# sharinka0715/semantic-gaussians

Measured on NVIDIA B200. Metric: Mviews/s + HBM GB/s, 1M Gaussians, 256-ch features, 1080p, fwd+bwd, higher is better.
Workload: dtype f32

## Files before the change

### semantic-gaussians_b200/csrc/blend_v3.cu

```cuda
#include <cstdlib>
#include <cstring>
#include <cuda.h>
#include "common.cuh"
#include "blend_pool.cuh"

namespace sgb {

namespace {

constexpr int kThreads = SGB_TILE_PIX;

__device__ __forceinline__ int lane_group8(int lane) { return (lane & 1) | (((lane >> 2) & 3) << 1); }
__device__ __forceinline__ int lane_group4(int lane) { return ((lane >> 1) & 1) | ((lane >> 4) << 1); }

template <int N>
__device__ __forceinline__ void xreduce_step(float (&v)[8], int lane, int step) {
    const bool upper = (lane & step) != 0;
#pragma unroll
    for (int i = 0; i < N / 2; i++) {
        const float send = upper ? v[i] : v[i + N / 2];
        const float keep = upper ? v[i + N / 2] : v[i];
        v[i] = keep + __shfl_xor_sync(0xffffffffu, send, step);
    }
}

constexpr int kAB = 32;

struct __align__(16) AlphaSmem {
    float4 recA[kAB];
    float4 recB[kAB];
    uint32_t ids[kAB];
    float wbuf[kAB][SGB_TILE_PIX];
    uint32_t wmask[8];
    uint32_t slot_chunk[kAB];
    uint32_t cur_chunk;
    uint32_t s_last;
};

template <bool DEPTH>
__global__ void __launch_bounds__(kThreads) alpha_pass_kernel(
    const uint2* __restrict__ ranges, const uint32_t* __restrict__ point_list, int W, int H,
    const SplatRec* __restrict__ rec, float* __restrict__ final_T, uint32_t* __restrict__ n_contrib,
    uint32_t* __restrict__ tile_last, float* __restrict__ out_depth, PoolView pool) {
    extern __shared__ __align__(128) unsigned char smem_raw[];
    AlphaSmem& sm = *reinterpret_cast<AlphaSmem*>(smem_raw);

    const int tiles_x = (W + SGB_TILE - 1) / SGB_TILE;
    const int tile = blockIdx.x;
    const int tid = threadIdx.x, lane = tid & 31, warp = tid >> 5;
    const uint32_t tx = tid & (SGB_TILE - 1), ty = tid >> 4;
    const uint2 pix = {(uint32_t)(tile % tiles_x) * SGB_TILE + tx, (uint32_t)(tile / tiles_x) * SGB_TILE + ty};
    const uint32_t pix_id = W * pix.y + pix.x;
    const float2 pixf = {(float)pix.x, (float)pix.y};
    const bool inside = pix.x < (uint32_t)W && pix.y < (uint32_t)H;
    bool done = !inside;

    const uint2 range = ranges[tile];
    const int total = (int)(range.y - range.x);
    const int nbatches = (total + kAB - 1) / kAB;
    const uint32_t dbase = range.x / kChunkEntries + (uint32_t)tile;
    if (tid == 0) { sm.cur_chunk = kNone; sm.s_last = 0; }

    float T = 1.0f;
    uint32_t last_contributor = 0;
    float D = 15.0f;
    uint32_t n_tile = 0;
    uint32_t n_blend = 0;

    auto load_id = [&](int bb) -> uint32_t {
        const int i = bb * kAB + tid;
        return (tid < kAB && bb < nbatches && i < total) ? __ldg(point_list + range.x + i) : 0u;
    };
    uint32_t id_cur = load_id(0), id_nxt = load_id(1);
    float4 rA = make_float4(0.f, 0.f, 0.f, 0.f), rB = rA;
    if (tid < kAB && tid < total) {
        const float4* rp = reinterpret_cast<const float4*>(rec + id_cur);
        rA = __ldg(rp);
        rB = __ldg(rp + 1);
    }
    for (int b = 0; b < nbatches; b++) {
        const int num_done = __syncthreads_count(done);
        if (num_done == kThreads) break;
        const int base = b * kAB;
        const int cnt = min(kAB, total - base);
        if (tid < cnt) {
            sm.ids[tid] = id_cur;
            sm.recA[tid] = rA;
            sm.recB[tid] = rB;
        }
        __syncthreads();
        if (tid < kAB) {
            id_cur = id_nxt;
            if (base + kAB + tid < total) {
                const float4* rp = reinterpret_cast<const float4*>(rec + id_cur);
                rA = __ldg(rp);
                rB = __ldg(rp + 1);
            }
            id_nxt = load_id(b + 2);
        }
        uint32_t my_mask = 0;
        for (int j = 0; j < cnt; j++) {
            float w = 0.f;
            if (!done) {
                const float4 a = sm.recA[j];
                const float2 xy = {a.x, a.y};
                const float2 d = {xy.x - pixf.x, xy.y - pixf.y};
                const float4 con_o = sm.recB[j];
                const float power = -0.5f * (con_o.x * d.x * d.x + con_o.z * d.y * d.y) - con_o.y * d.x * d.y;
                if (!(power > 0.0f)) {
                    const float alpha = min(0.99f, con_o.w * exp(power));
                    if (!(alpha < 1.0f / 255.0f)) {
                        const float test_T = T * (1 - alpha);
                        if (test_T < 0.0001f) {
                            done = true;
                        } else {
                            w = alpha * T;
                            if (DEPTH) {
                                if (T > 0.5f && test_T < 0.5) D = a.z;
                            }
                            T = test_T;
                            last_contributor = (uint32_t)(base + j + 1);
                        }
                    }
                }
            }
            sm.wbuf[j][tid] = w;
            n_blend += (w != 0.f);
            if (__ballot_sync(0xffffffffu, w != 0.f)) my_mask |= 1u << j;
        }
        if (lane == 0) sm.wmask[warp] = my_mask;
        __syncthreads();
        uint32_t tm = 0;
#pragma unroll
        for (int q = 0; q < 8; q++) tm |= sm.wmask[q];
        const int n_act = __popc(tm);
        if (n_act) {
            if (tid == 0) {
                uint32_t e = n_tile, cur = sm.cur_chunk;
                for (int k = 0; k < n_act; k++, e++) {
                    if ((e & (kChunkEntries - 1)) == 0) {
                        uint32_t nw = atomicAdd(&pool.hdr->counter, 1u);
                        if (nw >= pool.capacity) {
                            pool.hdr->overflow = 1;
                            nw = pool.capacity - 1;
                        }
                        pool.dir[dbase + e / kChunkEntries] = nw;
                        cur = nw;
                    }
                    sm.slot_chunk[k] = cur;
                }
                sm.cur_chunk = cur;
            }
            __syncthreads();
            int k = 0;
            for (uint32_t m = tm; m; m &= m - 1, k++) {
                const int j = __ffs(m) - 1;
                const uint32_t e = n_tile + k;
                WChunk& ck = pool.chunks[sm.slot_chunk[k]];
                const int s = e & (kChunkEntries - 1);
                ck.w[s][tid] = sm.wbuf[j][tid];
                if (tid == 0) {
                    uint32_t strips = 0;
#pragma unroll
                    for (int q = 0; q < 8; q++) strips |= ((sm.wmask[q] >> j) & 1u) << q;
                    ck.meta[s] = make_uint2(sm.ids[j], strips);
                }
// ... 199 lines not shown
    struct Stage {
        float w[ES][SGB_TILE_PIX];
        float f[ES][CH];
    };
    extern __shared__ __align__(128) unsigned char smem_raw[];
    Stage* stg = reinterpret_cast<Stage*>(smem_raw);
    __shared__ uint64_t full_bar[NS], empty_bar[NS];
    __shared__ uint32_t Cdir[kDirCap];
    __shared__ __align__(16) float Tsm[SGB_TILE_PIX];
    __shared__ float bgS[CH];

    const int tiles_x = (W + SGB_TILE - 1) / SGB_TILE;
    const int nchunksC = (C + CH - 1) / CH;
    const int tile = blockIdx.x / nchunksC;
    const int ch0 = (blockIdx.x % nchunksC) * CH;
    const int nch = min(CH, C - ch0);
    const int tid = threadIdx.x, lane = tid & 31, warp = tid >> 5;
    const int pg = lane_group4(lane), cg = lane_group8(lane);
    const uint2 pix_min = {(uint32_t)(tile % tiles_x) * SGB_TILE, (uint32_t)(tile / tiles_x) * SGB_TILE};

    const uint32_t n = pool.count[tile];
    const int nb = (int)((n + ES - 1) / ES);
    const uint32_t dbase = pool.dirbase[tile];
    if (tid == 0) {
        for (int i = 0; i < NS; i++) {
            mbar_init(&full_bar[i], 1);
            mbar_init(&empty_bar[i], kThreads / 32);
        }
        mbar_fence_init();
    }
    for (int k = tid; k < min(nb, kDirCap); k += kThreads) Cdir[k] = chunk_of(pool, dbase, k);
    {
        const uint32_t x = pix_min.x + (tid & (SGB_TILE - 1)), y = pix_min.y + (tid >> 4);
        Tsm[tid] = (x < (uint32_t)W && y < (uint32_t)H) ? final_T[(size_t)W * y + x] : 0.f;
        if (tid < nch) bgS[tid] = bg_color[ch0 + tid];
    }
    if (nch < CH)
        for (int e = tid; e < NS * ES * CH; e += kThreads) {
            const int k = e % CH;
            if (k >= nch) stg[e / (ES * CH)].f[(e / CH) % ES][k] = 0.f;
        }
    __syncthreads();

    auto chunk_ptr = [&](int bi) {
        return pool.chunks + (bi < kDirCap ? Cdir[bi] : chunk_of(pool, dbase, bi));
    };
    auto load_meta = [&](int bi) {
        uint2 m = make_uint2(0u, 0u);
        if (bi < nb && lane < min(ES, (int)n - bi * ES)) m = __ldg(&chunk_ptr(bi)->meta[lane]);
        return m;
    };
    auto issue = [&](int bi, uint2 meta) {
        const int st = bi % NS;
        const int cnt = min(ES, (int)n - bi * ES);
        if (bi >= NS) mbar_wait(&empty_bar[st], (uint32_t)(((bi / NS) - 1) & 1));
        if (lane < cnt) {
            const WChunk* ck = chunk_ptr(bi);
            bulk_g2s(&stg[st].w[lane][0], &ck->w[lane][0], SGB_TILE_PIX * 4u, &full_bar[st]);
            bulk_g2s(&stg[st].f[lane][0], features + (size_t)meta.x * C + ch0, (uint32_t)nch * 4u, &full_bar[st]);
        }
        __syncwarp();
        if (lane == 0) mbar_arrive_expect_tx(&full_bar[st], (uint32_t)cnt * (SGB_TILE_PIX * 4u + (uint32_t)nch * 4u));
    };
    uint2 meta_next = make_uint2(0u, 0u);
    int pb = 0;
    if (warp == 0) {
        uint2 m[LA];
#pragma unroll
        for (int i = 0; i < LA; i++) m[i] = load_meta(i);
#pragma unroll
        for (int i = 0; i < LA; i++)
            if (i < nb) issue(i, m[i]);
        pb = min(LA, nb);
        meta_next = load_meta(pb);
    }

    float2 acc[8][MCH / 2];
#pragma unroll
    for (int i = 0; i < 8; i++)
#pragma unroll
        for (int k = 0; k < MCH / 2; k++) acc[i][k] = make_float2(0.f, 0.f);

    const int woff = warp * 32 + pg * 8;
    auto entry = [&](const Stage& sg, int e) {
        const float4 w0 = *reinterpret_cast<const float4*>(&sg.w[e][woff]);
        const float4 w1 = *reinterpret_cast<const float4*>(&sg.w[e][woff + 4]);
        float2 f[MCH / 2];
#pragma unroll
        for (int q = 0; q < MCH / 4; q++) {
            const float4 t = *reinterpret_cast<const float4*>(&sg.f[e][q * 32 + cg * 4]);
            f[2 * q] = make_float2(t.x, t.y);
            f[2 * q + 1] = make_float2(t.z, t.w);
        }
        const float wv[8] = {w0.x, w0.y, w0.z, w0.w, w1.x, w1.y, w1.z, w1.w};
#pragma unroll
        for (int i = 0; i < 8; i++) {
            const float2 w2 = make_float2(wv[i], wv[i]);
#pragma unroll
            for (int k = 0; k < MCH / 2; k++) acc[i][k] = ffma2(f[k], w2, acc[i][k]);
        }
    };
    for (int b = 0; b < nb; b++) {
        const int st = b % NS;
        const int cnt = min(ES, (int)n - b * ES);
        if (warp == 0 && pb < nb) {
            issue(pb, meta_next);
            pb++;
            meta_next = load_meta(pb);
        }
        mbar_wait(&full_bar[st], (uint32_t)((b / NS) & 1));
        if (cnt == ES) {
#pragma unroll
            for (int e = 0; e < ES; e++) entry(stg[st], e);
        } else {
            for (int e = 0; e < cnt; e++) entry(stg[st], e);
        }
        __syncwarp();
        if (lane == 0) mbar_arrive(&empty_bar[st]);
    }
    const uint32_t row = pix_min.y + 2 * warp + (pg >> 1);
    const uint32_t col0 = pix_min.x + (pg & 1) * 8;
    if (acc_nonfinite<MCH>(acc)) {
        forward_redo_guarded<MCH, true>(pool, n, dbase, features, C, ch0, nch, warp, woff, cg, bg_color, final_T, W, H,
                                        row, col0, out_color);
        return;
    }
    if (row < (uint32_t)H) {
        const size_t plane = (size_t)H * W;
        const bool vec = ((W & 3) == 0) && (col0 + 8 <= (uint32_t)W);
        const float4 t0 = *reinterpret_cast<const float4*>(&Tsm[(2 * warp + (pg >> 1)) * SGB_TILE + (pg & 1) * 8]);
        const float4 t1 = *reinterpret_cast<const float4*>(&Tsm[(2 * warp + (pg >> 1)) * SGB_TILE + (pg & 1) * 8 + 4]);
        const float Tv[8] = {t0.x, t0.y, t0.z, t0.w, t1.x, t1.y, t1.z, t1.w};
#pragma unroll
        for (int k = 0; k < MCH; k++) {
            const int chl = (k >> 2) * 32 + cg * 4 + (k & 3);
            if (chl >= nch) continue;
            const float bgc = bgS[chl];
            float* dst = out_color + (size_t)(ch0 + chl) * plane + (size_t)W * row + col0;
            float o[8];
#pragma unroll
            for (int i = 0; i < 8; i++) o[i] = ((k & 1) ? acc[i][k / 2].y : acc[i][k / 2].x) + Tv[i] * bgc;
            if (vec) {
                reinterpret_cast<float4*>(dst)[0] = make_float4(o[0], o[1], o[2], o[3]);
                reinterpret_cast<float4*>(dst)[1] = make_float4(o[4], o[5], o[6], o[7]);
            } else {
#pragma unroll
                for (int i = 0; i < 8; i++)
                    if (col0 + i < (uint32_t)W) dst[i] = o[i];
            }
        }
    }
}

template <int CH>
__global__ void __launch_bounds__(kThreads, 2) dfeature_gemm_kernel(int W, int H, int C,
                                                                   const float* __restrict__ dL_dpixels,
                                                                   PoolView pool, float* __restrict__ dL_dcolors) {
    static_assert(CH == 64, "64-channel chunks");
    constexpr int DP = SGB_TILE_PIX;
    constexpr int WP = 36;
    extern __shared__ __align__(128) unsigned char smem_raw[];
    float(*dLs)[DP] = reinterpret_cast<float(*)[DP]>(smem_raw);
    float* wslab = reinterpret_cast<float*>(smem_raw + sizeof(float) * CH * DP);
    __shared__ const float* Wrow[128];
    __shared__ uint32_t Gid[128];

    const int tiles_x = (W + SGB_TILE - 1) / SGB_TILE;
    const int nchunksC = (C + CH - 1) / CH;
    const int tile = blockIdx.x / nchunksC;
    const int ch0 = (blockIdx.x % nchunksC) * CH;
    const int nch = min(CH, C - ch0);
    const int tid = threadIdx.x, lane = tid & 31, warp = tid >> 5;
    const uint32_t n = pool.count[tile];
    if (n == 0) return;
    const uint32_t dbase = __ldg(pool.dirbase + tile);
    const uint2 pix_min = {(uint32_t)(tile % tiles_x) * SGB_TILE, (uint32_t)(tile / tiles_x) * SGB_TILE};
    const size_t plane = (size_t)H * W;
    const bool rows16 = (W & 3) == 0 && (reinterpret_cast<uintptr_t>(dL_dpixels) & 15) == 0;
    for (int idx = tid; idx < CH * SGB_TILE * 4; idx += kThreads) {
        const int pc = idx & 3, r = (idx >> 2) & (SGB_TILE - 1), c = idx >> 6;
        const uint32_t y = pix_min.y + r, x = pix_min.x + pc * 4;
        float* dst = &dLs[c][((r * 4 + pc) ^ ((c >> 2) & 7)) * 4];
        const float* src = dL_dpixels + (size_t)(ch0 + c) * plane + (size_t)W * y + x;
        const bool rowok = c < nch && y < (uint32_t)H;
        if (rows16) {
            const bool ok = rowok && x + 4 <= (uint32_t)W;
            cp_async16(dst, ok ? src : dL_dpixels, ok ? 16 : 0);
        } else {
#pragma unroll
            for (int i = 0; i < 4; i++) dst[i] = (rowok && x + i < (uint32_t)W) ? __ldg(src + i) : 0.f;
        }
    }
    cp_async_commit();

    const int eg = lane_group4(lane), cg = lane_group8(lane);
    const bool red16 = ((C & 3) == 0) && ((reinterpret_cast<uintptr_t>(dL_dcolors) & 15) == 0);
    for (uint32_t base = 0; base < n; base += 128) {
        const int cnt = (int)min(128u, n - base);
        __syncthreads();
        if (tid < cnt) {
            const WChunk* ck = pool.chunks + chunk_of(pool, dbase, (int)((base + tid) / kChunkEntries));
            const int s = (base + tid) & (kChunkEntries - 1);
            Wrow[tid] = &ck->w[s][0];
            Gid[tid] = ck->meta[s].x;
        }
        cp_async_wait<0>();
        __syncthreads();
        if (warp * 16 < cnt) {
            float(*wsl)[16][WP] = reinterpret_cast<float(*)[16][WP]>(wslab + (size_t)warp * 2 * 16 * WP);
            const float* lrow[4];
#pragma unroll
            for (int i = 0; i < 4; i++) lrow[i] = Wrow[min(warp * 16 + (lane >> 3) + 4 * i, cnt - 1)] + (lane & 7) * 4;
            auto issue = [&](int sl, int buf) {
#pragma unroll
                for (int i = 0; i < 4; i++)
                    cp_async16(&wsl[buf][(lane >> 3) + 4 * i][(lane & 7) * 4], lrow[i] + sl * 32, 16);
                cp_async_commit();
            };
            float2 acc[4][8];
#pragma unroll
            for (int j = 0; j < 4; j++)
#pragma unroll
                for (int k = 0; k < 8; k++) acc[j][k] = make_float2(0.f, 0.f);
            issue(0, 0);
            for (int sl = 0; sl < SGB_TILE_PIX / 32; sl++) {
                const int buf = sl & 1;
                if (sl + 1 < SGB_TILE_PIX / 32) { issue(sl + 1, buf ^ 1); cp_async_wait<1>(); }
                else cp_async_wait<0>();
                __syncwarp();
                const float* drow = &dLs[4 * cg][0];
                const float* wbase = &wsl[buf][eg][0];
                auto ld_d = [&](int step) {
                    const int k = step & 7, p4 = step >> 3;
                    return *reinterpret_cast<const float4*>(drow + ((k >> 2) * 32 + (k & 3)) * DP +
                                                            (((sl * 8 + p4) ^ cg) << 2));
                };
                float4 wq[4], wn[4];
#pragma unroll
                for (int j = 0; j < 4; j++) wq[j] = *reinterpret_cast<const float4*>(wbase + 4 * j * WP);
                float4 d0 = ld_d(0), d1 = ld_d(1);
#pragma unroll
                for (int p4 = 0; p4 < 8; p4++) {
#pragma unroll
                    for (int k = 0; k < 8; k++) {
                        const int step = p4 * 8 + k;
                        float4 d2 = d1;
                        if (step + 2 < 64) d2 = ld_d(step + 2);
                        if (k == 2 && p4 + 1 < 8) {
#pragma unroll
                            for (int j = 0; j < 4; j++)
                                wn[j] = *reinterpret_cast<const float4*>(wbase + 4 * j * WP + (p4 + 1) * 4);
                        }
#pragma unroll
                        for (int j = 0; j < 4; j++) {
                            acc[j][k] = ffma2(make_float2(wq[j].x, wq[j].y), make_float2(d0.x, d0.y), acc[j][k]);
                            acc[j][k] = ffma2(make_float2(wq[j].z, wq[j].w), make_float2(d0.z, d0.w), acc[j][k]);
                        }
                        d0 = d1;
                        d1 = d2;
                    }
                    if (p4 + 1 < 8) {
#pragma unroll
                        for (int j = 0; j < 4; j++) wq[j] = wn[j];
                    }
                }
                __syncwarp();
            }
#pragma unroll
            for (int j = 0; j < 4; j++) {
                const int e = warp * 16 + eg + 4 * j;
                if (e < cnt) {
                    float* dst = dL_dcolors + (size_t)Gid[e] * C + ch0 + 4 * cg;
#pragma unroll
                    for (int h = 0; h < 2; h++) {
                        const int chl = h * 32 + 4 * cg;
                        const float4 v = make_float4(acc[j][4 * h + 0].x + acc[j][4 * h + 0].y, acc[j][4 * h + 1].x + acc[j][4 * h + 1].y,
                                                     acc[j][4 * h + 2].x + acc[j][4 * h + 2].y, acc[j][4 * h + 3].x + acc[j][4 * h + 3].y);
                        if (red16 && chl + 4 <= nch) {
                            red_add_v4_f32(dst + h * 32, v);
                        } else {
                            if (chl + 0 < nch) red_add_f32(dst + h * 32 + 0, v.x);
                            if (chl + 1 < nch) red_add_f32(dst + h * 32 + 1, v.y);
                            if (chl + 2 < nch) red_add_f32(dst + h * 32 + 2, v.z);
                            if (chl + 3 < nch) red_add_f32(dst + h * 32 + 3, v.w);
                        }
                    }
                }
            }
        }
    }
}

template <bool VEC>
__global__ void __launch_bounds__(kThreads, 2) chain_backward_gemm_kernel(
    int W, int H, int C, const float* __restrict__ bg_color, const SplatRec* __restrict__ rec,
    const float* __restrict__ features, const float* __restrict__ final_Ts, const float* __restrict__ dL_dpixels,
    PoolView pool, float* __restrict__ dL_dmean2D, float* __restrict__ dL_dconic2D, float* __restrict__ dL_dopacity) {
    constexpr int CK = 16;
    constexpr int FP = kSeg + 4;
    extern __shared__ __align__(128) unsigned char smem_raw[];
    float(*S)[kSeg][32] = reinterpret_cast<float(*)[kSeg][32]>(smem_raw);
    float(*FT)[CK][FP] = reinterpret_cast<float(*)[CK][FP]>(smem_raw + sizeof(float) * 8 * kSeg * 32);
    float(*DS)[2][CK][32] = reinterpret_cast<float(*)[2][CK][32]>(
        smem_raw + sizeof(float) * (8 * kSeg * 32 + 2 * CK * FP));
    __shared__ const float* Wrow[kSeg];
    __shared__ uint2 Meta[kSeg];
    __shared__ float4 RecA[kSeg], RecB[kSeg];

    const int tiles_x = (W + SGB_TILE - 1) / SGB_TILE;
    const int tile = blockIdx.x;
    const int tid = threadIdx.x, lane = tid & 31, warp = tid >> 5;
    const int pg = lane >> 3, eg = lane & 7;
    const uint2 pix_min = {(uint32_t)(tile % tiles_x) * SGB_TILE, (uint32_t)(tile / tiles_x) * SGB_TILE};
    const uint32_t tx = tid & (SGB_TILE - 1), ty = tid >> 4;
    const uint2 pix = {pix_min.x + tx, pix_min.y + ty};
    const uint32_t pix_id = W * pix.y + pix.x;
    const float2 pixf = {(float)pix.x, (float)pix.y};
    const bool inside = pix.x < (uint32_t)W && pix.y < (uint32_t)H;
    const uint32_t n = pool.count[tile];
    if (n == 0) return;
    const uint32_t dbase = pool.dirbase[tile];

    const size_t plane = (size_t)H * W;
    const bool rows16 = ((W & 3) == 0) && ((reinterpret_cast<uintptr_t>(dL_dpixels) & 15) == 0);
    const int woff = warp * 32 + lane;

    int bg_nonzero = 0;
    for (int ch = tid; ch < C; ch += kThreads) bg_nonzero |= (bg_color[ch] != 0.f);
    bg_nonzero = __syncthreads_or(bg_nonzero);
    float bgdot = 0.f;
    if (inside && bg_nonzero)
        for (int ch = 0; ch < C; ch++) bgdot += bg_color[ch] * __ldg(dL_dpixels + (size_t)ch * plane + pix_id);

    const float T_final = inside ? final_Ts[pix_id] : 0.f;
    float T = T_final;
    float last_alpha = 0.f, s_last = 0.f, A = 0.f;
    const float ddelx_dx = 0.5f * W, ddely_dy = 0.5f * H;

    const int nseg = (int)((n + kSeg - 1) / kSeg);
    for (int sg = nseg - 1; sg >= 0; sg--) {
        const int base = sg * kSeg;
        const int cnt = min(kSeg, (int)n - base);
        __syncthreads();
        if (tid < kSeg) {
            if (tid < cnt) {
                const WChunk* ck = pool.chunks + chunk_of(pool, dbase, (base + tid) / kChunkEntries);
                const int s = (base + tid) & (kChunkEntries - 1);
                Wrow[tid] = &ck->w[s][0];
                const uint2 mt = ck->meta[s];
                Meta[tid] = mt;
                const float4* rp = reinterpret_cast<const float4*>(rec + mt.x);
                RecA[tid] = __ldg(rp);
                RecB[tid] = __ldg(rp + 1);
            } else {
                Meta[tid] = make_uint2(0u, 0u);
            }
        }
        __syncthreads();

        float2 acc[8][4];
#pragma unroll
        for (int i = 0; i < 8; i++)
#pragma unroll
            for (int j = 0; j < 4; j++) acc[i][j] = make_float2(0.f, 0.f);

        const int nslab = (C + CK - 1) / CK;
        float4 fpre;
        auto fload = [&](int sl) {
            const int e = tid >> 2, q = tid & 3;
            const int chb = sl * CK + q * 4;
            fpre = make_float4(0.f, 0.f, 0.f, 0.f);
            if (e < cnt) {
                const float* src = features + (size_t)Meta[e].x * C + chb;
                if (VEC && chb + 4 <= C) fpre = __ldg(reinterpret_cast<const float4*>(src));
                else {
                    if (chb < C) fpre.x = __ldg(src);
                    if (chb + 1 < C) fpre.y = __ldg(src + 1);
                    if (chb + 2 < C) fpre.z = __ldg(src + 2);
                    if (chb + 3 < C) fpre.w = __ldg(src + 3);
                }
            }
        };
        auto fstore = [&](int buf) {
            const int e = tid >> 2, q = tid & 3;
            const int pos = ((e >> 3) << 2) | (e & 3) | (((e >> 2) & 1) << 5);
            FT[buf][q * 4 + 0][pos] = fpre.x;
            FT[buf][q * 4 + 1][pos] = fpre.y;
            FT[buf][q * 4 + 2][pos] = fpre.z;
            FT[buf][q * 4 + 3][pos] = fpre.w;
        };
        auto dissue = [&](int sl, int buf) {
#pragma unroll
            for (int i = 0; i < CK / 4; i++) {
                const int chl = (lane >> 3) + 4 * i;
                const int ch = sl * CK + chl;
                const int pc = lane & 7;
                const uint32_t y = pix_min.y + 2 * warp + (pc >> 2);
                const uint32_t x = pix_min.x + (pc & 3) * 4;
                const bool rowin = ch < C && y < (uint32_t)H;
                const float* src = dL_dpixels + (size_t)ch * plane + (size_t)W * y + x;
                if (rows16) {
                    const bool ok = rowin && x + 4 <= (uint32_t)W;
                    cp_async16(&DS[warp][buf][chl][pc * 4], ok ? src : dL_dpixels, ok ? 16 : 0);
                } else {
#pragma unroll
                    for (int u = 0; u < 4; u++)
                        DS[warp][buf][chl][pc * 4 + u] = (rowin && x + u < (uint32_t)W) ? __ldg(src + u) : 0.f;
                }
            }
            cp_async_commit();
        };
        fload(0);
        dissue(0, 0);
        fstore(0);
        if (nslab > 1) fload(1);
        for (int sl = 0; sl < nslab; sl++) {
            const int buf = sl & 1;
            if (sl + 1 < nslab) { dissue(sl + 1, buf ^ 1); cp_async_wait<1>(); }
            else cp_async_wait<0>();
            __syncthreads();
#pragma unroll 4
            for (int k = 0; k < CK; k++) {
                const float4 d0 = *reinterpret_cast<const float4*>(&DS[warp][buf][k][pg * 8]);
                const float4 d1 = *reinterpret_cast<const float4*>(&DS[warp][buf][k][pg * 8 + 4]);
                const float4 f0 = *reinterpret_cast<const float4*>(&FT[buf][k][eg * 4]);
                const float4 f1 = *reinterpret_cast<const float4*>(&FT[buf][k][32 + eg * 4]);
                const float2 ff[4] = {make_float2(f0.x, f0.y), make_float2(f0.z, f0.w), make_float2(f1.x, f1.y),
                                      make_float2(f1.z, f1.w)};
                const float d[8] = {d0.x, d0.y, d0.z, d0.w, d1.x, d1.y, d1.z, d1.w};
#pragma unroll
                for (int i = 0; i < 8; i++) {
                    const float2 d2 = make_float2(d[i], d[i]);
#pragma unroll
                    for (int j = 0; j < 4; j++) acc[i][j] = ffma2(ff[j], d2, acc[i][j]);
                }
            }
            if (sl + 1 < nslab) {
                fstore(buf ^ 1);
                if (sl + 2 < nslab) fload(sl + 2);
            }
            __syncwarp();
        }
#pragma unroll
// ... 635 lines not shown
    return guess;
}

static int launch_alpha_pass(sgb_ctx* ctx, const sgb_view_inputs& in, GeomView g, BinView b, ImgView im,
                             float* out_depth, const PoolView& pv, cudaStream_t s) {
    const int tiles = num_tiles(in);
    const size_t smem = sizeof(AlphaSmem);
    static DeviceOnce attr_set;
    if (attr_set.first_use_on_device()) {
        SGB_CUDA(cudaFuncSetAttribute(alpha_pass_kernel<false>, cudaFuncAttributeMaxDynamicSharedMemorySize, (int)smem));
        SGB_CUDA(cudaFuncSetAttribute(alpha_pass_kernel<true>, cudaFuncAttributeMaxDynamicSharedMemorySize, (int)smem));
    }
    SGB_CUDA(cudaMemsetAsync(pv.hdr, 0, sizeof(PoolHdr), s));
    StageTimer t(ctx, ST_ALPHA, s);
    if (out_depth)
        alpha_pass_kernel<true><<<tiles, kThreads, smem, s>>>(im.ranges, b.point_list, in.W, in.H, g.rec, im.final_T,
                                                            im.n_contrib, im.tile_last, out_depth, pv);
    else
        alpha_pass_kernel<false><<<tiles, kThreads, smem, s>>>(im.ranges, b.point_list, in.W, in.H, g.rec, im.final_T,
                                                             im.n_contrib, im.tile_last, nullptr, pv);
    SGB_LAUNCH_CHECK("alpha_pass_kernel", in.debug, s);
    ctx->launches += 1;
    return SGB_OK;
}

static int launch_forward_gemm(sgb_ctx* ctx, const sgb_view_inputs& in, ImgView im, const float* colors,
                               float* out_color, const PoolView& pv, cudaStream_t s) {
    const int tiles = num_tiles(in);
    const int chunks = (in.C + 63) / 64;
    const bool vec = (in.C % 4 == 0) && ((reinterpret_cast<uintptr_t>(colors) & 15) == 0);
    if (vec && blend_mma_enabled()) return launch_forward_mma(ctx, in, im, colors, out_color, pv, s);
    static const bool use_warp = [] { const char* e = getenv("SGB_FWD_WARP"); return e && e[0] == '1'; }();
    StageTimer t(ctx, ST_BLEND_FWD, s);
    ctx->launches += 1;
    if (use_warp) {
        const int nslices = (in.C + 31) / 32;
        const int SL = nslices >= 4 ? 4 : nslices;
        const int groups = (nslices + SL - 1) / SL;
        const size_t smem_w = sizeof(FwdWarpSmem) * (kThreads / 32);
        if (vec)
            blend_forward_warp_kernel<true><<<tiles * groups, kThreads, smem_w, s>>>(in.W, in.H, in.C, SL, colors, in.background,
                                                                                    im.final_T, pv, out_color);
        else
            blend_forward_warp_kernel<false><<<tiles * groups, kThreads, smem_w, s>>>(in.W, in.H, in.C, SL, colors, in.background,
                                                                                     im.final_T, pv, out_color);
        SGB_LAUNCH_CHECK("blend_forward_warp_kernel", in.debug, s);
        return SGB_OK;
    }
    if (vec) {
        constexpr int NS = 5;
        const size_t smem_f = (size_t)NS * kChunkEntries * (SGB_TILE_PIX + 64) * sizeof(float);
        static DeviceOnce fattr;
        if (fattr.first_use_on_device()) {
            SGB_CUDA(cudaFuncSetAttribute(blend_forward_tma_kernel<64, NS>, cudaFuncAttributeMaxDynamicSharedMemorySize,
                                          (int)smem_f));
        }
        blend_forward_tma_kernel<64, NS><<<tiles * chunks, kThreads, smem_f, s>>>(in.W, in.H, in.C, colors, in.background,
                                                                                  im.final_T, pv, out_color);
    } else {
        blend_forward_v3_kernel<64, false><<<tiles * chunks, kThreads, 0, s>>>(in.W, in.H, in.C, colors, in.background,
                                                                                   im.final_T, pv, out_color);
    }
    SGB_LAUNCH_CHECK("blend_forward kernel", in.debug, s);
    return SGB_OK;
}

static inline PoolHdr* pinned_hdr(sgb_ctx* ctx, int view_slot) {
    return reinterpret_cast<PoolHdr*>(reinterpret_cast<char*>(ctx->pinned) + 8 * kMaxBatch) + view_slot;
}

int blend_forward_v3_alpha(sgb_ctx* ctx, int view_slot, const sgb_view_inputs& in, int64_t R, GeomView g, BinView b,
                           ImgView im, cudaStream_t s) {
    const int tiles = num_tiles(in);
    PoolSlot* sl = pool_acquire(ctx, b);
    uint64_t want = pool_first_guess(ctx, tiles, R);
    if (sl->chunks > want && sl->mem.cap >= pool_bytes(tiles, sl->chunks, R, nullptr, nullptr)) want = sl->chunks;
    const uint32_t chunks = (uint32_t)want;
    int rc = sl->mem.ensure(pool_bytes(tiles, chunks, R, nullptr, nullptr));
    if (rc) return rc;
    sl->chunks = chunks;
    PoolView pv;
    pool_bytes(tiles, chunks, R, &pv, sl->mem.p);
    rc = launch_alpha_pass(ctx, in, g, b, im, nullptr, pv, s);
    if (rc) return rc;
    SGB_CUDA(cudaMemcpyAsync(pinned_hdr(ctx, view_slot), pv.hdr, sizeof(PoolHdr), cudaMemcpyDeviceToHost, s));
    return SGB_OK;
}

int blend_forward_v3_gemm(sgb_ctx* ctx, const sgb_view_inputs& in, int64_t R, BinView b, ImgView im,
                          const float* colors, float* out_color, cudaStream_t s) {
    PoolSlot* sl = pool_find(ctx, in, R, b);
    if (!sl) { set_error("forward GEMM without validated weight rows"); return SGB_E_INVALID; }
    PoolView pv;
    pool_bytes(num_tiles(in), sl->chunks, R, &pv, sl->mem.p);
    return launch_forward_gemm(ctx, in, im, colors, out_color, pv, s);
}

int blend_forward_v3_finish(sgb_ctx* ctx, int view_slot, const sgb_view_inputs& in, int64_t R, BinView b) {
    PoolSlot* sl = nullptr;
    for (PoolSlot& c : ctx->pools)
        if (c.key_bin == (const void*)b.point_list) { sl = &c; break; }
    if (!sl) { set_error("weight-pool slot of the view vanished"); return SGB_E_INVALID; }
    const PoolHdr h = *pinned_hdr(ctx, view_slot);
    if (h.overflow) {
        const uint64_t need = (uint64_t)h.counter + h.counter / 8 + 64;
        if (need > ctx->pool_chunks_hint) ctx->pool_chunks_hint = need;
        sl->chunks = 0;
        return 1;
    }
    ctx->stat_blended_pairs = (int64_t)h.blended;
    ctx->stat_pool_chunks = h.counter;
    if (h.counter > ctx->pool_chunks_hint) ctx->pool_chunks_hint = (uint64_t)h.counter + h.counter / 16 + 16;
    sl->valid = true;
    sl->key_R = R;
    sl->key_W = in.W;
    sl->key_H = in.H;
    sl->key_P = in.P;
    return 0;
}

static int pool_for_backward(sgb_ctx* ctx, const sgb_view_inputs& in, int64_t R, GeomView g, BinView b, ImgView im,
                             PoolView* pv, cudaStream_t s) {
    const int tiles = num_tiles(in);
    if (PoolSlot* hit = pool_find(ctx, in, R, b)) {
        pool_bytes(tiles, hit->chunks, R, pv, hit->mem.p);
        return SGB_OK;
    }
    for (int attempt = 0; attempt < 4; attempt++) {
        PoolSlot* sl = pool_acquire(ctx, b);
        const uint32_t chunks = (uint32_t)pool_first_guess(ctx, tiles, R);
        int rc = sl->mem.ensure(pool_bytes(tiles, chunks, R, nullptr, nullptr));
        if (rc) return rc;
        sl->chunks = chunks;
        pool_bytes(tiles, chunks, R, pv, sl->mem.p);
        rc = launch_alpha_pass(ctx, in, g, b, im, nullptr, *pv, s);
        if (rc) return rc;
        SGB_CUDA(cudaMemcpyAsync(pinned_hdr(ctx, 0), pv->hdr, sizeof(PoolHdr), cudaMemcpyDeviceToHost, s));
        SGB_CUDA(cudaStreamSynchronize(s));
        rc = blend_forward_v3_finish(ctx, 0, in, R, b);
        if (rc <= 0) return rc;
    }
    set_error("weight pool kept overflowing");
    return SGB_E_NOMEM;
}

int blend_backward_v3_dfeature(sgb_ctx* ctx, const sgb_view_inputs& in, int64_t R, GeomView g, BinView b, ImgView im,
                               const float* dL_dpix, float* dL_dcolors, cudaStream_t s) {
    PoolView pv;
    int rc = pool_for_backward(ctx, in, R, g, b, im, &pv, s);
    if (rc) return rc;
    if (blend_mma_enabled() && in.C % 4 == 0 && (reinterpret_cast<uintptr_t>(dL_dcolors) & 15) == 0)
        return launch_dfeature_mma(ctx, in, dL_dpix, dL_dcolors, pv, s);
    const int tiles = num_tiles(in);
    const int chunks = (in.C + 63) / 64;
    const size_t smem_d = sizeof(float) * (64 * SGB_TILE_PIX + 8 * 2 * 16 * 36);
    static DeviceOnce attr_set;
    if (attr_set.first_use_on_device())
        SGB_CUDA(cudaFuncSetAttribute(dfeature_gemm_kernel<64>, cudaFuncAttributeMaxDynamicSharedMemorySize, (int)smem_d));
    StageTimer t(ctx, ST_DFEATURE, s);
    ctx->launches += 1;
    dfeature_gemm_kernel<64><<<tiles * chunks, kThreads, smem_d, s>>>(in.W, in.H, in.C, dL_dpix, pv, dL_dcolors);
    SGB_LAUNCH_CHECK("dfeature_gemm_kernel", in.debug, s);
    return SGB_OK;
}

static bool encode_dl_map(CUtensorMap* map, const float* dL_dpix, int W, int H, int C) {
    using EncodeFn = CUresult (*)(CUtensorMap*, CUtensorMapDataType, cuuint32_t, void*, const cuuint64_t*, const cuuint64_t*,
                                  const cuuint32_t*, const cuuint32_t*, CUtensorMapInterleave, CUtensorMapSwizzle,
                                  CUtensorMapL2promotion, CUtensorMapFloatOOBfill);
    static const EncodeFn encode = [] {
        void* fn = nullptr;
        cudaDriverEntryPointQueryResult q;
        if (cudaGetDriverEntryPoint("cuTensorMapEncodeTiled", &fn, cudaEnableDefault, &q) != cudaSuccess ||
            q != cudaDriverEntryPointSuccess)
            fn = nullptr;
        return (EncodeFn)fn;
    }();
    memset(map, 0, sizeof(*map));
    const char* off = getenv("SGB_CHAIN_TMA");
    if (off && off[0] == '0') return false;
    if (!encode || (W & 3) != 0 || (reinterpret_cast<uintptr_t>(dL_dpix) & 15) != 0) return false;
    const cuuint64_t dims[3] = {(cuuint64_t)W, (cuuint64_t)H, (cuuint64_t)C};
    const cuuint64_t strides[2] = {(cuuint64_t)W * sizeof(float), (cuuint64_t)W * H * sizeof(float)};
    const cuuint32_t box[3] = {SGB_TILE, 2, 16};
    const cuuint32_t estr[3] = {1, 1, 1};
    return encode(map, CU_TENSOR_MAP_DATA_TYPE_FLOAT32, 3, const_cast<float*>(dL_dpix), dims, strides, box, estr,
                  CU_TENSOR_MAP_INTERLEAVE_NONE, CU_TENSOR_MAP_SWIZZLE_NONE, CU_TENSOR_MAP_L2_PROMOTION_L2_128B,
                  CU_TENSOR_MAP_FLOAT_OOB_FILL_NONE) == CUDA_SUCCESS;
}

int blend_backward_v3_chain(sgb_ctx* ctx, const sgb_view_inputs& in, int64_t R, GeomView g, BinView b, ImgView im,
                            const float* colors, const float* dL_dpix, float* dL_dmean2D, float* dL_dconic,
                            float* dL_dopacity, cudaStream_t s) {
    PoolView pv;
    int rc = pool_for_backward(ctx, in, R, g, b, im, &pv, s);
    if (rc) return rc;
    const int tiles = num_tiles(in);
    const bool vec = (in.C % 4 == 0) && ((reinterpret_cast<uintptr_t>(colors) & 15) == 0);
    if (vec && blend_mma_enabled())
        return launch_chain_mma(ctx, in, g, im, colors, dL_dpix, dL_dmean2D, dL_dconic, dL_dopacity, pv, s);
    static const bool use_v3 = [] { const char* e = getenv("SGB_CHAIN_V3"); return e && e[0] == '1'; }();
    const size_t smem_g = sizeof(float) * (8 * kSeg * 32 + 2 * 16 * (kSeg + 4) + 8 * 2 * 16 * 32);
    const size_t smem_w = sizeof(ChainWarpSmem) * (kThreads / 32);
    static DeviceOnce attr_set;
    if (attr_set.first_use_on_device()) {
        SGB_CUDA(cudaFuncSetAttribute(chain_backward_gemm_kernel<true>, cudaFuncAttributeMaxDynamicSharedMemorySize, (int)smem_g));
        SGB_CUDA(cudaFuncSetAttribute(chain_backward_gemm_kernel<false>, cudaFuncAttributeMaxDynamicSharedMemorySize, (int)smem_g));
        SGB_CUDA(cudaFuncSetAttribute(chain_backward_warp_kernel<true>, cudaFuncAttributeMaxDynamicSharedMemorySize, (int)smem_w));
        SGB_CUDA(cudaFuncSetAttribute(chain_backward_warp_kernel<false>, cudaFuncAttributeMaxDynamicSharedMemorySize, (int)smem_w));
    }
    StageTimer t(ctx, ST_BLEND_BWD, s);
    ctx->launches += 1;
#define SGB_CHAIN_ARGS in.W, in.H, in.C, in.background, g.rec, colors, im.final_T, dL_dpix, pv, dL_dmean2D, dL_dconic, dL_dopacity
    if (use_v3) {
        if (vec) chain_backward_gemm_kernel<true><<<tiles, kThreads, smem_g, s>>>(SGB_CHAIN_ARGS);
        else chain_backward_gemm_kernel<false><<<tiles, kThreads, smem_g, s>>>(SGB_CHAIN_ARGS);
    } else {
        CUtensorMap dl_map;
        const int use_tma = encode_dl_map(&dl_map, dL_dpix, in.W, in.H, in.C) ? 1 : 0;
        if (vec) chain_backward_warp_kernel<true><<<tiles, kThreads, smem_w, s>>>(SGB_CHAIN_ARGS, dl_map, use_tma);
        else chain_backward_warp_kernel<false><<<tiles, kThreads, smem_w, s>>>(SGB_CHAIN_ARGS, dl_map, use_tma);
    }
#undef SGB_CHAIN_ARGS
    SGB_LAUNCH_CHECK("chain backward kernel", in.debug, s);
    return SGB_OK;
}

}
```

Measured before the change: 0.00008634.

## Restructure dfeature kernel into staged plan with TMA bulk loads and split-K warps

Replaces the per-(tile,channel-chunk) dfeature GEMM kernel with one block per tile that walks all channel chunks and entry rounds as a sequence of half-tile stages. Each stage's dL/dpixel slice is fetched with bulk async copies into a double buffer guarded by mbarriers, so the next stage loads while the current one computes. When a round has few entry groups, several warps split the pixel slabs of one group so idle warps are used. The catch is fewer blocks in the grid, more barrier synchronisation per stage, and a more complex schedule. This path runs only when the MMA path is disabled.

```diff
diff --git a/semantic-gaussians_b200/csrc/blend_v3.cu b/semantic-gaussians_b200/csrc/blend_v3.cu
--- a/semantic-gaussians_b200/csrc/blend_v3.cu
+++ b/semantic-gaussians_b200/csrc/blend_v3.cu
@@ -3,6 +3,7 @@
 #include <cuda.h>
 #include "common.cuh"
 #include "blend_pool.cuh"
+#include "dfeature_plan.cuh"
 
 namespace sgb {
 
@@ -10,8 +11,8 @@
 
 constexpr int kThreads = SGB_TILE_PIX;
 
-__device__ __forceinline__ int lane_group8(int lane) { return (lane & 1) | (((lane >> 2) & 3) << 1); }
-__device__ __forceinline__ int lane_group4(int lane) { return ((lane >> 1) & 1) | ((lane >> 4) << 1); }
+using dfp::lane_group8;
+using dfp::lane_group4;
 
 template <int N>
 __device__ __forceinline__ void xreduce_step(float (&v)[8], int lane, int step) {
@@ -517,143 +518,199 @@
     }
 }
 
-template <int CH>
-__global__ void __launch_bounds__(kThreads, 2) dfeature_gemm_kernel(int W, int H, int C,
-                                                                   const float* __restrict__ dL_dpixels,
-                                                                   PoolView pool, float* __restrict__ dL_dcolors) {
-    static_assert(CH == 64, "64-channel chunks");
-    constexpr int DP = SGB_TILE_PIX;
-    constexpr int WP = 36;
-    extern __shared__ __align__(128) unsigned char smem_raw[];
-    float(*dLs)[DP] = reinterpret_cast<float(*)[DP]>(smem_raw);
-    float* wslab = reinterpret_cast<float*>(smem_raw + sizeof(float) * CH * DP);
-    __shared__ const float* Wrow[128];
-    __shared__ uint32_t Gid[128];
-
-    const int tiles_x = (W + SGB_TILE - 1) / SGB_TILE;
-    const int nchunksC = (C + CH - 1) / CH;
-    const int tile = blockIdx.x / nchunksC;
-    const int ch0 = (blockIdx.x % nchunksC) * CH;
-    const int nch = min(CH, C - ch0);
-    const int tid = threadIdx.x, lane = tid & 31, warp = tid >> 5;
-    const uint32_t n = pool.count[tile];
+struct DfeatureOps {
+    static constexpr int kSlabOff = 2 * dfp::kBufFloats * 4;
+    static constexpr int kRowOff = kSlabOff + dfp::kWarps * dfp::kWSlabFloats * 4;
+    static constexpr int kGidOff = kRowOff + dfp::kRoundEntries * 8;
+    static constexpr int kBarOff = kGidOff + dfp::kRoundEntries * 4;
+    static constexpr int kTileOff = kBarOff + 2 * 8;
+    static constexpr int kPlanOff = kTileOff + 2 * 4;
+    static constexpr int kSmemBytes = kPlanOff + (int)sizeof(dfp::Plan);
+    static __device__ __forceinline__ unsigned char* smem() {
+        extern __shared__ __align__(128) unsigned char smem_raw[];
+        return smem_raw;
+    }
+    static __device__ __forceinline__ float* dls() { return reinterpret_cast<float*>(smem()); }
+    static __device__ __forceinline__ float* wsl() {
+        return reinterpret_cast<float*>(smem() + kSlabOff) + (threadIdx.x >> 5) * dfp::kWSlabFloats;
+    }
+    static __device__ __forceinline__ const float** Wrow() { return reinterpret_cast<const float**>(smem() + kRowOff); }
+    static __device__ __forceinline__ uint32_t* Gid() { return reinterpret_cast<uint32_t*>(smem() + kGidOff); }
+    static __device__ __forceinline__ uint64_t* bar() { return reinterpret_cast<uint64_t*>(smem() + kBarOff); }
+    static __device__ __forceinline__ uint32_t* tile_n_dbase() { return reinterpret_cast<uint32_t*>(smem() + kTileOff); }
+    static __device__ __forceinline__ dfp::Plan& plan() { return *reinterpret_cast<dfp::Plan*>(smem() + kPlanOff); }
+
+    int W, H, C;
+    const float* __restrict__ dL;
+    PoolView pool;
+    float* __restrict__ out;
+    float2 acc[4][8];
+
+    __device__ __forceinline__ void sync() { __syncthreads(); }
+
+    __device__ __forceinline__ void rows(int round) {
+        const int base = round * dfp::kRoundEntries;
+        const int cnt = min(dfp::kRoundEntries, (int)tile_n_dbase()[0] - base);
+        const uint32_t dbase = tile_n_dbase()[1];
+        const int tid = threadIdx.x;
+        if (tid < cnt) {
+            const WChunk* ck = pool.chunks + chunk_of(pool, dbase, (base + tid) / kChunkEntries);
+            const int s = (base + tid) & (kChunkEntries - 1);
+            Wrow()[tid] = &ck->w[s][0];
+            Gid()[tid] = ck->meta[s].x;
+        }
+    }
+
+    __device__ __forceinline__ void issue(int k) {
+        const dfp::Stage st = dfp::stage_of(plan(), k);
+        const int tid = threadIdx.x;
+        const int tiles_x = (W + SGB_TILE - 1) / SGB_TILE;
+        const int x0 = (int)(blockIdx.x % tiles_x) * SGB_TILE;
+        const size_t plane = (size_t)H * W;
+        const bool bulk = (W & 3) == 0 && (reinterpret_cast<uintptr_t>(dL) & 15) == 0;
+        float* buf = dls() + (k & 1) * dfp::kBufFloats;
+        uint64_t* kbar = &bar()[k & 1];
+        const int ch0 = st.chunk * dfp::kCh, nch = min(dfp::kCh, C - ch0);
+        const int y0 = (int)(blockIdx.x / tiles_x) * SGB_TILE + st.half * 8;
+        const int rv = max(0, min(8, H - y0));
+        const int cw = max(0, min(SGB_TILE, W - x0));
+        const float4 z = make_float4(0.f, 0.f, 0.f, 0.f);
+        if (bulk) {
+            if (tid == 0) mbar_arrive_expect_tx(kbar, (uint32_t)(nch * rv * cw * 4));
+            fence_proxy_async_smem();
+            for (int p = tid; p < dfp::kPiecesPerStage; p += kThreads) {
+                const int c = dfp::piece_ch(p), r = dfp::piece_row(p);
+                float* dst = buf + dfp::dl_off(c, r * 4);
+                const bool in = c < nch && r < rv;
+                if (in)
+                    bulk_g2s(dst, dL + (size_t)(ch0 + c) * plane + (size_t)W * (y0 + r) + x0, (uint32_t)cw * 4, kbar);
+                for (int q = in ? cw / 4 : 0; q < 4; q++) reinterpret_cast<float4*>(dst)[q] = z;
+            }
+        } else {
+            for (int p = tid; p < dfp::kPiecesPerStage; p += kThreads) {
+                const int c = dfp::piece_ch(p), r = dfp::piece_row(p);
+                float* dst = buf + dfp::dl_off(c, r * 4);
+                const bool in = c < nch && r < rv;
+                const float* src = dL + (size_t)(ch0 + min(c, nch - 1)) * plane + (size_t)W * (y0 + min(r, max(rv - 1, 0))) + x0;
+#pragma unroll
+                for (int i = 0; i < SGB_TILE; i++) dst[i] = (in && i < cw) ? __ldg(src + i) : 0.f;
+            }
+            if (tid == 0) mbar_arrive(kbar);
+        }
+    }
+
+    __device__ __forceinline__ void wait(int k) { mbar_wait(&bar()[k & 1], (uint32_t)(k >> 1) & 1u); }
+
+    __device__ __forceinline__ void unit(int ks, const dfp::Stage& st, const dfp::Unit& u) {
+        constexpr int WP = dfp::kWPitch;
+        const int base = st.round * dfp::kRoundEntries;
+        const int cnt = min(dfp::kRoundEntries, (int)tile_n_dbase()[0] - base);
+        const int gl = u.group * dfp::kGroup - base;
+        const int nsl = dfp::kSlabsPerStage / u.nsplit;
+        const int lane = threadIdx.x & 31, eg = dfp::lane_group4(lane), cg = dfp::lane_group8(lane);
+        const float* dbuf = dls() + (ks & 1) * dfp::kBufFloats;
+        float* const wsl = DfeatureOps::wsl();
+        const float* const* Wrow = DfeatureOps::Wrow();
+        auto issue_w = [&](int i, int b) {
+            const int px = st.half * dfp::kStagePx + (u.split + u.nsplit * i) * dfp::kSlabPx + (lane & 7) * 4;
+#pragma unroll
+            for (int r = 0; r < 4; r++) {
+                const int e = (lane >> 3) + 4 * r;
+                const float* row = Wrow[min(gl + e, cnt - 1)];
+                cp_async16(wsl + dfp::w_off(b, e, (lane & 7) * 4), row + px, 16);
+            }
+            cp_async_commit();
+        };
+        if (st.half == 0) {
+#pragma unroll
+            for (int j = 0; j < 4; j++)
+#pragma unroll
+                for (int k = 0; k < 8; k++) acc[j][k] = make_float2(0.f, 0.f);
+        }
+        issue_w(0, 0);
+#pragma unroll 1
+        for (int i = 0; i < nsl; i++) {
+            const int b = i & 1;
+            if (i + 1 < nsl) { issue_w(i + 1, b ^ 1); cp_async_wait<1>(); }
+            else cp_async_wait<0>();
+            __syncwarp();
+            const int sl = u.split + u.nsplit * i;
+            const float* drow = dbuf + dfp::dl_off(dfp::chan_of(cg, 0), dfp::quad_of(sl, 0));
+            const float* wbase = wsl + dfp::w_off(b, eg, 0);
+            auto ld_d = [&](int step) {
+                return *reinterpret_cast<const float4*>(drow + dfp::dl_step(step & 7, step >> 3));
+            };
+            float4 wq[4], wn[4];
+#pragma unroll
+            for (int j = 0; j < 4; j++) wq[j] = *reinterpret_cast<const float4*>(wbase + 4 * j * WP);
+            float4 d0 = ld_d(0), d1 = ld_d(1);
+#pragma unroll 1
+            for (int p4 = 0; p4 < 8; p4++) {
+#pragma unroll
+                for (int k = 0; k < 8; k++) {
+                    const float4 d2 = ld_d(p4 * 8 + k + 2);
+                    if (k >= 4)
+                        wn[k - 4] = *reinterpret_cast<const float4*>(wbase + 4 * (k - 4) * WP + (p4 + 1) * 4);
+#pragma unroll
+                    for (int j = 0; j < 4; j++) {
+                        acc[j][k] = ffma2(make_float2(wq[j].x, wq[j].y), make_float2(d0.x, d0.y), acc[j][k]);
+                        acc[j][k] = ffma2(make_float2(wq[j].z, wq[j].w), make_float2(d0.z, d0.w), acc[j][k]);
+                    }
+                    d0 = d1;
+                    d1 = d2;
+                }
+#pragma unroll
+                for (int j = 0; j < 4; j++) wq[j] = wn[j];
+            }
+            __syncwarp();
+        }
+        if (st.half == 0) return;
+        const bool red16 = ((C & 3) == 0) && ((reinterpret_cast<uintptr_t>(out) & 15) == 0);
+        const int ch0 = st.chunk * dfp::kCh, nch = min(dfp::kCh, C - ch0);
+#pragma unroll
+        for (int j = 0; j < 4; j++) {
+            const int e = gl + dfp::entry_of(eg, j);
+            if (e < cnt) {
+                float* dst = out + (size_t)Gid()[e] * C + ch0 + 4 * cg;
+#pragma unroll
+                for (int h = 0; h < 2; h++) {
+                    const int chl = dfp::chan_of(cg, 4 * h);
+                    const float4 v = make_float4(acc[j][4 * h + 0].x + acc[j][4 * h + 0].y, acc[j][4 * h + 1].x + acc[j][4 * h + 1].y,
+                                                 acc[j][4 * h + 2].x + acc[j][4 * h + 2].y, acc[j][4 * h + 3].x + acc[j][4 * h + 3].y);
+                    if (red16 && chl + 4 <= nch) {
+                        red_add_v4_f32(dst + h * 32, v);
+                    } else {
+                        if (chl + 0 < nch) red_add_f32(dst + h * 32 + 0, v.x);
+                        if (chl + 1 < nch) red_add_f32(dst + h * 32 + 1, v.y);
+                        if (chl + 2 < nch) red_add_f32(dst + h * 32 + 2, v.z);
+                        if (chl + 3 < nch) red_add_f32(dst + h * 32 + 3, v.w);
+                    }
+                }
+            }
+        }
+    }
+};
+
+__global__ void __launch_bounds__(kThreads, 2) dfeature_kernel(int W, int H, int C, const float* __restrict__ dL_dpixels,
+                                                              PoolView pool, float* __restrict__ dL_dcolors) {
+    const uint32_t n = pool.count[blockIdx.x];
     if (n == 0) return;
-    const uint32_t dbase = __ldg(pool.dirbase + tile);
-    const uint2 pix_min = {(uint32_t)(tile % tiles_x) * SGB_TILE, (uint32_t)(tile / tiles_x) * SGB_TILE};
-    const size_t plane = (size_t)H * W;
-    const bool rows16 = (W & 3) == 0 && (reinterpret_cast<uintptr_t>(dL_dpixels) & 15) == 0;
-    for (int idx = tid; idx < CH * SGB_TILE * 4; idx += kThreads) {
-        const int pc = idx & 3, r = (idx >> 2) & (SGB_TILE - 1), c = idx >> 6;
-        const uint32_t y = pix_min.y + r, x = pix_min.x + pc * 4;
-        float* dst = &dLs[c][((r * 4 + pc) ^ ((c >> 2) & 7)) * 4];
-        const float* src = dL_dpixels + (size_t)(ch0 + c) * plane + (size_t)W * y + x;
-        const bool rowok = c < nch && y < (uint32_t)H;
-        if (rows16) {
-            const bool ok = rowok && x + 4 <= (uint32_t)W;
-            cp_async16(dst, ok ? src : dL_dpixels, ok ? 16 : 0);
-        } else {
-#pragma unroll
-            for (int i = 0; i < 4; i++) dst[i] = (rowok && x + i < (uint32_t)W) ? __ldg(src + i) : 0.f;
-        }
-    }
-    cp_async_commit();
-
-    const int eg = lane_group4(lane), cg = lane_group8(lane);
-    const bool red16 = ((C & 3) == 0) && ((reinterpret_cast<uintptr_t>(dL_dcolors) & 15) == 0);
-    for (uint32_t base = 0; base < n; base += 128) {
-        const int cnt = (int)min(128u, n - base);
-        __syncthreads();
-        if (tid < cnt) {
-            const WChunk* ck = pool.chunks + chunk_of(pool, dbase, (int)((base + tid) / kChunkEntries));
-            const int s = (base + tid) & (kChunkEntries - 1);
-            Wrow[tid] = &ck->w[s][0];
-            Gid[tid] = ck->meta[s].x;
-        }
-        cp_async_wait<0>();
-        __syncthreads();
-        if (warp * 16 < cnt) {
-            float(*wsl)[16][WP] = reinterpret_cast<float(*)[16][WP]>(wslab + (size_t)warp * 2 * 16 * WP);
-            const float* lrow[4];
-#pragma unroll
-            for (int i = 0; i < 4; i++) lrow[i] = Wrow[min(warp * 16 + (lane >> 3) + 4 * i, cnt - 1)] + (lane & 7) * 4;
-            auto issue = [&](int sl, int buf) {
-#pragma unroll
-                for (int i = 0; i < 4; i++)
-                    cp_async16(&wsl[buf][(lane >> 3) + 4 * i][(lane & 7) * 4], lrow[i] + sl * 32, 16);
-                cp_async_commit();
-            };
-            float2 acc[4][8];
-#pragma unroll
-            for (int j = 0; j < 4; j++)
-#pragma unroll
-                for (int k = 0; k < 8; k++) acc[j][k] = make_float2(0.f, 0.f);
-            issue(0, 0);
-            for (int sl = 0; sl < SGB_TILE_PIX / 32; sl++) {
-                const int buf = sl & 1;
-                if (sl + 1 < SGB_TILE_PIX / 32) { issue(sl + 1, buf ^ 1); cp_async_wait<1>(); }
-                else cp_async_wait<0>();
-                __syncwarp();
-                const float* drow = &dLs[4 * cg][0];
-                const float* wbase = &wsl[buf][eg][0];
-                auto ld_d = [&](int step) {
-                    const int k = step & 7, p4 = step >> 3;
-                    return *reinterpret_cast<const float4*>(drow + ((k >> 2) * 32 + (k & 3)) * DP +
-                                                            (((sl * 8 + p4) ^ cg) << 2));
-                };
-                float4 wq[4], wn[4];
-#pragma unroll
-                for (int j = 0; j < 4; j++) wq[j] = *reinterpret_cast<const float4*>(wbase + 4 * j * WP);
-                float4 d0 = ld_d(0), d1 = ld_d(1);
-#pragma unroll
-                for (int p4 = 0; p4 < 8; p4++) {
-#pragma unroll
-                    for (int k = 0; k < 8; k++) {
-                        const int step = p4 * 8 + k;
-                        float4 d2 = d1;
-                        if (step + 2 < 64) d2 = ld_d(step + 2);
-                        if (k == 2 && p4 + 1 < 8) {
-#pragma unroll
-                            for (int j = 0; j < 4; j++)
-                                wn[j] = *reinterpret_cast<const float4*>(wbase + 4 * j * WP + (p4 + 1) * 4);
-                        }
-#pragma unroll
-                        for (int j = 0; j < 4; j++) {
-                            acc[j][k] = ffma2(make_float2(wq[j].x, wq[j].y), make_float2(d0.x, d0.y), acc[j][k]);
-                            acc[j][k] = ffma2(make_float2(wq[j].z, wq[j].w), make_float2(d0.z, d0.w), acc[j][k]);
-                        }
-                        d0 = d1;
-                        d1 = d2;
-                    }
-                    if (p4 + 1 < 8) {
-#pragma unroll
-                        for (int j = 0; j < 4; j++) wq[j] = wn[j];
-                    }
-                }
-                __syncwarp();
-            }
-#pragma unroll
-            for (int j = 0; j < 4; j++) {
-                const int e = warp * 16 + eg + 4 * j;
-                if (e < cnt) {
-                    float* dst = dL_dcolors + (size_t)Gid[e] * C + ch0 + 4 * cg;
-#pragma unroll
-                    for (int h = 0; h < 2; h++) {
-                        const int chl = h * 32 + 4 * cg;
-                        const float4 v = make_float4(acc[j][4 * h + 0].x + acc[j][4 * h + 0].y, acc[j][4 * h + 1].x + acc[j][4 * h + 1].y,
-                                                     acc[j][4 * h + 2].x + acc[j][4 * h + 2].y, acc[j][4 * h + 3].x + acc[j][4 * h + 3].y);
-                        if (red16 && chl + 4 <= nch) {
-                            red_add_v4_f32(dst + h * 32, v);
-                        } else {
-                            if (chl + 0 < nch) red_add_f32(dst + h * 32 + 0, v.x);
-                            if (chl + 1 < nch) red_add_f32(dst + h * 32 + 1, v.y);
-                            if (chl + 2 < nch) red_add_f32(dst + h * 32 + 2, v.z);
-                            if (chl + 3 < nch) red_add_f32(dst + h * 32 + 3, v.w);
-                        }
-                    }
-                }
-            }
-        }
-    }
+    DfeatureOps ops;
+    ops.W = W;
+    ops.H = H;
+    ops.C = C;
+    ops.dL = dL_dpixels;
+    ops.pool = pool;
+    ops.out = dL_dcolors;
+    if (threadIdx.x == 0) {
+        DfeatureOps::plan() = dfp::make_plan(n, C);
+        DfeatureOps::tile_n_dbase()[0] = n;
+        DfeatureOps::tile_n_dbase()[1] = __ldg(pool.dirbase + blockIdx.x);
+        mbar_init(&DfeatureOps::bar()[0], 1);
+        mbar_init(&DfeatureOps::bar()[1], 1);
+        mbar_fence_init();
+    }
+    dfp::walk(DfeatureOps::plan(), (int)(threadIdx.x >> 5), ops);
 }
 
 template <bool VEC>
@@ -1595,15 +1652,14 @@
     if (blend_mma_enabled() && in.C % 4 == 0 && (reinterpret_cast<uintptr_t>(dL_dcolors) & 15) == 0)
         return launch_dfeature_mma(ctx, in, dL_dpix, dL_dcolors, pv, s);
     const int tiles = num_tiles(in);
-    const int chunks = (in.C + 63) / 64;
-    const size_t smem_d = sizeof(float) * (64 * SGB_TILE_PIX + 8 * 2 * 16 * 36);
+    const size_t smem_d = DfeatureOps::kSmemBytes;
     static DeviceOnce attr_set;
     if (attr_set.first_use_on_device())
-        SGB_CUDA(cudaFuncSetAttribute(dfeature_gemm_kernel<64>, cudaFuncAttributeMaxDynamicSharedMemorySize, (int)smem_d));
+        SGB_CUDA(cudaFuncSetAttribute(dfeature_kernel, cudaFuncAttributeMaxDynamicSharedMemorySize, (int)smem_d));
     StageTimer t(ctx, ST_DFEATURE, s);
     ctx->launches += 1;
-    dfeature_gemm_kernel<64><<<tiles * chunks, kThreads, smem_d, s>>>(in.W, in.H, in.C, dL_dpix, pv, dL_dcolors);
-    SGB_LAUNCH_CHECK("dfeature_gemm_kernel", in.debug, s);
+    dfeature_kernel<<<tiles, kThreads, smem_d, s>>>(in.W, in.H, in.C, dL_dpix, pv, dL_dcolors);
+    SGB_LAUNCH_CHECK("dfeature_kernel", in.debug, s);
     return SGB_OK;
 }
 
diff --git a/semantic-gaussians_b200/csrc/dfeature_plan.cuh b/semantic-gaussians_b200/csrc/dfeature_plan.cuh
--- /dev/null
+++ b/semantic-gaussians_b200/csrc/dfeature_plan.cuh
@@ -0,0 +1,107 @@
+#pragma once
+#include <cstdint>
+
+#ifdef __CUDACC__
+#define SGB_DFP_HD __host__ __device__ __forceinline__
+#else
+#define SGB_DFP_HD inline
+#endif
+
+namespace sgb {
+namespace dfp {
+
+constexpr int kWarps = 8;
+constexpr int kCh = 64;
+constexpr int kGroup = 16;
+constexpr int kRoundGroups = 8;
+constexpr int kRoundEntries = kGroup * kRoundGroups;
+constexpr int kStagePx = 128;
+constexpr int kSlabPx = 32;
+constexpr int kSlabsPerStage = kStagePx / kSlabPx;
+constexpr int kQuads = kStagePx / 4;
+constexpr int kBufFloats = kCh * kStagePx + (kCh / 4) * 4;
+constexpr int kPiecesPerStage = kCh * (kStagePx / 16);
+constexpr int kWPitch = 36;
+constexpr int kWSlabFloats = 2 * kGroup * kWPitch;
+
+struct Plan {
+    int groups;
+    int rounds;
+    int chunks;
+    int stages;
+};
+
+SGB_DFP_HD Plan make_plan(uint32_t n, int C) {
+    Plan p;
+    p.groups = (int)((n + kGroup - 1) / kGroup);
+    p.rounds = (p.groups + kRoundGroups - 1) / kRoundGroups;
+    p.chunks = (C + kCh - 1) / kCh;
+    p.stages = p.chunks * p.rounds * 2;
+    return p;
+}
+
+struct Stage {
+    int chunk, round, half;
+};
+
+SGB_DFP_HD Stage stage_of(const Plan& p, int k) {
+    Stage s;
+    s.half = k & 1;
+    s.round = (k >> 1) % p.rounds;
+    s.chunk = (k >> 1) / p.rounds;
+    return s;
+}
+
+SGB_DFP_HD int splits_for(int g) { return g >= 5 ? 1 : (g >= 3 ? 2 : 4); }
+
+struct Unit {
+    bool active;
+    int group;
+    int split;
+    int nsplit;
+};
+
+SGB_DFP_HD Unit unit_of(const Plan& p, int round, int warp) {
+    const int rem = p.groups - round * kRoundGroups;
+    const int g = rem < kRoundGroups ? rem : kRoundGroups;
+    Unit u;
+    u.nsplit = splits_for(g);
+    u.active = warp < g * u.nsplit;
+    u.group = round * kRoundGroups + warp / u.nsplit;
+    u.split = warp % u.nsplit;
+    return u;
+}
+
+SGB_DFP_HD int lane_group8(int lane) { return (lane & 1) | (((lane >> 2) & 3) << 1); }
+SGB_DFP_HD int lane_group4(int lane) { return ((lane >> 1) & 1) | ((lane >> 4) << 1); }
+SGB_DFP_HD int entry_of(int eg, int j) { return eg + 4 * j; }
+SGB_DFP_HD int chan_of(int cg, int k) { return (k >> 2) * 32 + 4 * cg + (k & 3); }
+
+SGB_DFP_HD int dl_off(int ch, int q) { return ch * kStagePx + (ch >> 2) * 4 + q * 4; }
+SGB_DFP_HD int dl_step(int k, int p4) { return ((k >> 2) * 32 + (k & 3)) * kStagePx + (k >> 2) * 32 + p4 * 4; }
+SGB_DFP_HD int w_off(int buf, int e, int px) { return (buf * kGroup + e) * kWPitch + px; }
+SGB_DFP_HD int quad_of(int sl, int p4) { return sl * 8 + p4; }
+SGB_DFP_HD int piece_ch(int piece) { return piece >> 3; }
+SGB_DFP_HD int piece_row(int piece) { return piece & 7; }
+
+#ifdef __CUDACC__
+#pragma nv_exec_check_disable
+#endif
+template <class Ops>
+SGB_DFP_HD void walk(const Plan& p, int warp, Ops& ops) {
+    ops.sync();
+    if (p.stages > 0) ops.issue(0);
+    for (int k = 0; k < p.stages; k++) {
+        const Stage st = stage_of(p, k);
+        ops.sync();
+        if (st.half == 0 && (p.rounds > 1 || k == 0)) ops.rows(st.round);
+        if (k + 1 < p.stages) ops.issue(k + 1);
+        ops.wait(k);
+        ops.sync();
+        const Unit u = unit_of(p, st.round, warp);
+        if (u.active) ops.unit(k, st, u);
+    }
+}
+
+}
+}
```

Measured after the change: 0.00008458, median of 6. -2.0%, worse.
